# amazon-science/crossmodal-contrastive-learning

Hardware: AMD Instinct MI355X
Metric: contrastive-pairs/sec (fwd+bwd) (higher is better)
Workload: dtype bf16

## Files before the change

### crossmodal-contrastive-learning_amd/csrc/crossclr_api.cpp

```cpp
#include "../../include/crossclr.h"
#include "crossclr_kernels_generic.h"
#include "crossclr_kernels_hvp.h"
#include "crossclr_kernels_topk.h"
#ifndef CROSSCLR_NO_FAST
#include "crossclr_kernels_fast.h"
#include "crossclr_kernels_project.h"
#include "crossclr_kernels_saved32.h"
#endif

#include <math.h>
#include <stdarg.h>
#include <stdio.h>
#include <stdlib.h>
#include <string.h>
#include <type_traits>

#ifndef CROSSCLR_DEFAULT_BWD_KERNEL
#define CROSSCLR_DEFAULT_BWD_KERNEL 1
#endif

using namespace crossclr;

static thread_local char g_err[512] = "";

// ... 265 lines not shown

template <typename TIN, bool NORM>
static int normalize_t(const crossclr_plan* p, const void* v, const void* t, long ldv, long ldt, void* xhat,
                       float* inv_norm, float* diag, void* stream, int* zero_word) {
    Geo g; memset(&g, 0, sizeof(g));
    g.b = p->b; g.bpad = p->bpad; g.D = p->D; g.Dpad = p->Dpad;
    dim3 grid((p->bpad + 3) / 4), block(256);
    if (p->mode == CROSSCLR_MODE_FP32)
        LAUNCH((normalize_kernel<TIN, float, NORM>), grid, block, stream, (const TIN*)v, (const TIN*)t, ldv, ldt, g,
               (float*)xhat, inv_norm, diag, zero_word);
    else if (is_x3(p))
        LAUNCH((normalize_kernel<TIN, x3_t, NORM>), grid, block, stream, (const TIN*)v, (const TIN*)t, ldv, ldt, g,
               (x3_t*)xhat, inv_norm, diag, zero_word);
    else
        LAUNCH((normalize_kernel<TIN, bf16_t, NORM>), grid, block, stream, (const TIN*)v, (const TIN*)t, ldv, ldt, g,
               (bf16_t*)xhat, inv_norm, diag, zero_word);
    return launch_status("normalize_kernel");
}
template <bool NORM>
static int normalize_any(const crossclr_plan* plan, const void* video, const void* text, long ld_video, long ld_text, int in_dtype,
                         void* xhat, float* inv_norm, float* diag_cos, void* stream, int* zero_word = nullptr) {
    if (!plan || !video || !text || !xhat || !inv_norm || !diag_cos) return fail(CROSSCLR_E_ARG, "NULL argument");
    if (ld_video < plan->D || ld_text < plan->D) return fail(CROSSCLR_E_ARG, "row stride smaller than D");
    switch (in_dtype) {
        case CROSSCLR_IN_F32: return normalize_t<float, NORM>(plan, video, text, ld_video, ld_text, xhat, inv_norm, diag_cos, stream, zero_word);
        case CROSSCLR_IN_F64: return normalize_t<double, NORM>(plan, video, text, ld_video, ld_text, xhat, inv_norm, diag_cos, stream, zero_word);
        case CROSSCLR_IN_F16: return normalize_t<in_f16, NORM>(plan, video, text, ld_video, ld_text, xhat, inv_norm, diag_cos, stream, zero_word);
        case CROSSCLR_IN_BF16: return normalize_t<in_bf16, NORM>(plan, video, text, ld_video, ld_text, xhat, inv_norm, diag_cos, stream, zero_word);
    }
    return fail(CROSSCLR_E_ARG, "bad in_dtype %d", in_dtype);
}

#ifndef CROSSCLR_NO_FAST
template <typename TIN, bool NORM>
static int normalize_xf_t(const crossclr_plan* p, const void* v, const void* t, long ldv, long ldt, void* xhat, void* xf,
                          float* inv_norm, float* diag, void* stream, int* zero_word) {
    Geo g; memset(&g, 0, sizeof(g));
    g.b = p->b; g.bpad = p->bpad; g.D = p->D; g.Dpad = p->Dpad;
    if (p->Dpad <= 512)
        LAUNCH((normalize_xf_kernel<TIN, NORM, 2>), dim3(p->bpad / 16), dim3(512), stream, (const TIN*)v, (const TIN*)t, ldv, ldt, g,
               (bf16_t*)xhat, (unsigned char*)xf, inv_norm, diag, zero_word);
    else
        LAUNCH((normalize_xf_kernel<TIN, NORM, 4>), dim3(p->bpad / 16), dim3(512), stream, (const TIN*)v, (const TIN*)t, ldv, ldt, g,
               (bf16_t*)xhat, (unsigned char*)xf, inv_norm, diag, zero_word);
    return launch_status("normalize_xf_kernel");
}
#endif
template <bool NORM>
static int normalize_xf_any(const crossclr_plan* plan, const void* video, const void* text, long ld_video, long ld_text, int in_dtype,
                            void* xhat, void* xf, float* inv_norm, float* diag_cos, void* stream, int* zero_word = nullptr) {
    if (!plan || !video || !text || !xhat || !xf || !inv_norm || !diag_cos) return fail(CROSSCLR_E_ARG, "NULL argument");
    if (ld_video < plan->D || ld_text < plan->D) return fail(CROSSCLR_E_ARG, "row stride smaller than D");
#ifdef CROSSCLR_NO_FAST
    return fail(CROSSCLR_E_ARG, "the fragment-major operand needs the register-resident path");
#else
    if (!plan->xf_bytes) return fail(CROSSCLR_E_ARG, "this plan has no fragment-major operand (xf_bytes == 0): use crossclr_normalize / crossclr_pack");
    if (plan->Dpad > 1024) {
        if (int rc = normalize_any<NORM>(plan, video, text, ld_video, ld_text, in_dtype, xhat, inv_norm, diag_cos, stream, zero_word)) return rc;
        return crossclr_pack_xf_from_packed(plan, xhat, 1, xf, stream);
    }
    switch (in_dtype) {
        case CROSSCLR_IN_F32: return normalize_xf_t<float, NORM>(plan, video, text, ld_video, ld_text, xhat, xf, inv_norm, diag_cos, stream, zero_word);
        case CROSSCLR_IN_F64: return normalize_xf_t<double, NORM>(plan, video, text, ld_video, ld_text, xhat, xf, inv_norm, diag_cos, stream, zero_word);
        case CROSSCLR_IN_F16: return normalize_xf_t<in_f16, NORM>(plan, video, text, ld_video, ld_text, xhat, xf, inv_norm, diag_cos, stream, zero_word);
        case CROSSCLR_IN_BF16: return normalize_xf_t<in_bf16, NORM>(plan, video, text, ld_video, ld_text, xhat, xf, inv_norm, diag_cos, stream, zero_word);
    }
    return fail(CROSSCLR_E_ARG, "bad in_dtype %d", in_dtype);
#endif
}
extern "C" int crossclr_normalize_xf(const crossclr_plan* plan, const void* video, const void* text, long ld_video, long ld_text,
                                     int in_dtype, void* xhat, void* xhat_xf, float* inv_norm, float* diag_cos, void* stream) {
    return normalize_xf_any<true>(plan, video, text, ld_video, ld_text, in_dtype, xhat, xhat_xf, inv_norm, diag_cos, stream);
}
extern "C" int crossclr_pack_xf(const crossclr_plan* plan, const void* video_hat, const void* text_hat, long ld_video, long ld_text,
                                int in_dtype, void* xhat, void* xhat_xf, float* inv_norm, float* diag_cos, void* stream) {
    return normalize_xf_any<false>(plan, video_hat, text_hat, ld_video, ld_text, in_dtype, xhat, xhat_xf, inv_norm, diag_cos, stream);
}
// ... 433 lines not shown
        return fail(CROSSCLR_E_ARG, "slot0 must be L * plan->fwd_slots, L = 0..%d", kLaunchGroups - 1);
    const int n = 2 * plan->bpad;
    LAUNCH(fwd_add_kernel, dim3((n + 255) / 256), dim3(256), stream, vec, n, part + (size_t)slot0 * n,
           reinterpret_cast<int*>(part + ws_flag_off(plan)) + 4 * (slot0 / plan->fwd_slots));
    return launch_status("fwd_add_kernel");
}

extern "C" int crossclr_forward_finish(const crossclr_plan* plan, const float* part, int nslots,
                                       const float* diag_cos, float temperature, float negative_weight,
                                       float* logz, float* rz, float* wrz, double* loss_sum, void* stream) {
    return crossclr_forward_finish_w(plan, part, nslots, diag_cos, temperature, negative_weight, nullptr, logz, rz, wrz,
                                     loss_sum, stream);
}

extern "C" int crossclr_forward_finish_w(const crossclr_plan* plan, const float* part, int nslots,
                                         const float* diag_cos, float temperature, float negative_weight,
                                         const crossclr_sample_weights* sw, float* logz, float* rz, float* wrz,
                                         double* loss_sum, void* stream) {
    if (!plan || !part || !diag_cos || !logz || !rz || !wrz || !loss_sum || plan->fwd_slots <= 0 || nslots <= 0 ||
        nslots % plan->fwd_slots != 0 || nslots / plan->fwd_slots > kLaunchGroups)
        return fail(CROSSCLR_E_ARG, "NULL argument / nslots must be fwd_slots times the number of launch groups (1..%d)", kLaunchGroups);
    Geo g;
    int rc = make_geo(plan, 1, plan->rank, -1, temperature, negative_weight, &g);
    if (rc) return rc;
    const int nb = plan->loss_ws_doubles - 1;
    const int nlaunch = nslots / plan->fwd_slots;
    return crossclr_forward_finish_s(plan, part, nslots, diag_cos, temperature, negative_weight, sw, nullptr, logz, rz, wrz, loss_sum,
                                     stream);
}

static int forward_finish_impl(const crossclr_plan* plan, const float* part, int nslots,
                               const float* diag_cos, float temperature, float negative_weight,
                               const crossclr_sample_weights* sw, const float* shift_rows, float* logz, float* rz,
                               float* wrz, double* loss_sum, void* stream, int* ticket);
extern "C" int crossclr_forward_finish_s(const crossclr_plan* plan, const float* part, int nslots,
                                         const float* diag_cos, float temperature, float negative_weight,
                                         const crossclr_sample_weights* sw, const float* shift_rows, float* logz, float* rz,
                                         float* wrz, double* loss_sum, void* stream) {
    return forward_finish_impl(plan, part, nslots, diag_cos, temperature, negative_weight, sw, shift_rows, logz, rz, wrz, loss_sum, stream, nullptr);
}
static int forward_finish_impl(const crossclr_plan* plan, const float* part, int nslots,
                               const float* diag_cos, float temperature, float negative_weight,
                               const crossclr_sample_weights* sw, const float* shift_rows, float* logz, float* rz,
                               float* wrz, double* loss_sum, void* stream, int* ticket) {
    if (!plan || !part || !diag_cos || !logz || !rz || !wrz || !loss_sum || plan->fwd_slots <= 0 || nslots <= 0 ||
        nslots % plan->fwd_slots != 0 || nslots / plan->fwd_slots > kLaunchGroups)
        return fail(CROSSCLR_E_ARG, "NULL argument / nslots must be fwd_slots times the number of launch groups (1..%d)", kLaunchGroups);
    Geo g;
    int rc = make_geo(plan, 1, plan->rank, -1, temperature, negative_weight, &g, shift_rows != nullptr);
    if (rc) return rc;
    if ((g.row_shift != 0) != (shift_rows != nullptr))
        return fail(CROSSCLR_E_ARG, "shift_rows must be given exactly when crossclr_needs_row_shift(temperature, negative_weight)");
    const int nb = plan->loss_ws_doubles - 1;
    const int nlaunch = nslots / plan->fwd_slots;
    LAUNCH(fwd_finish_kernel, dim3(nb), dim3(256), stream, part, nlaunch, plan->fwd_slots, g, diag_cos, 1.0f / temperature,
           negative_weight, logz, rz, wrz, loss_sum, part + ws_colpart_off(plan),
           reinterpret_cast<const int*>(part + ws_flag_off(plan)), sw ? sw->neg_scale_rows : nullptr,
           sw ? sw->loss_weight : nullptr, shift_rows, ticket, 1.0 / (2.0 * (double)plan->b * (double)plan->world));
    if (!ticket) LAUNCH(fwd_finish_reduce_kernel, dim3(1), dim3(64), stream, loss_sum, nb, 1.0 / (2.0 * (double)plan->b * (double)plan->world));
    return launch_status("fwd_finish_kernel");
}

extern "C" int crossclr_needs_row_shift(float temperature, float negative_weight) {
    return (temperature > 0.f && isfinite(temperature) && isfinite(negative_weight) && needs_row_shift(temperature, negative_weight)) ? 1 : 0;
}

extern "C" int crossclr_forward_rowmax(const crossclr_plan* plan, const void* xhat_rows, const void* xhat_cols, int col_ranks,
                                       int col_rank0, int skip_rank, float temperature, float negative_weight,
                                       const crossclr_sample_weights* sw, float* part, float* shift_rows, int accumulate,
                                       void* stream) {
    if (!plan || !xhat_rows || !xhat_cols || !part || !shift_rows) return fail(CROSSCLR_E_ARG, "NULL argument");
    const float *krows, *kcols;
    if (int rk = unpack_k(sw, &krows, &kcols)) return rk;
    Geo g;
    int rc = make_geo(plan, col_ranks, col_rank0, skip_rank, temperature, negative_weight, &g, true);
    if (rc) return rc;
    const bool skipping = skip_rank >= col_rank0 && skip_rank < col_rank0 + col_ranks;
    const int n = 2 * plan->bpad;
    int nslots = plan->fwd_slots;
    const float* colpart = nullptr;
    if (col_ranks - (skipping ? 1 : 0) <= 0) nslots = 0;
    else if (xhat_rows == xhat_cols && col_ranks == 1 && col_rank0 == plan->rank && skip_rank < 0 && krows == kcols &&
             !env_knobs().disable_symmetric) {
        float* cp = part + ws_colpart_off(plan);
        int* header = reinterpret_cast<int*>(part + ws_flag_off(plan));
        rc = is_x3(plan) ? forward_generic_sym<x3_t>(plan, g, xhat_rows, part, kcols, cp, header, stream, nullptr, nullptr, true)
           : plan->mode == CROSSCLR_MODE_FP32 ? forward_generic_sym<float>(plan, g, xhat_rows, part, kcols, cp, header, stream, nullptr, nullptr, true)
                                              : forward_generic_sym<bf16_t>(plan, g, xhat_rows, part, kcols, cp, header, stream, nullptr, nullptr, true);
        if (rc) return rc;
        colpart = cp;
    } else if ((rc = forward_generic(plan, g, xhat_rows, xhat_cols, part, kcols, nullptr, 1, stream))) return rc;
// ... 1063 lines not shown
    if (int rc = step_bind(plan, layout, persistent, transient, true, &B)) return rc;
    const crossclr_step_layout& L = B.L;
    const float temperature = L.temperature, negative_weight = L.negative_weight;
    const unsigned flags = L.flags;
    const float* k = sw ? sw->neg_scale_rows : nullptr;
    const float* lw = sw ? sw->loss_weight : nullptr;
    const crossclr_sample_weights sw_k = {k, k, nullptr}, sw_klw = {k, k, lw};
    const crossclr_sample_weights* pk = k ? &sw_k : nullptr;
    const crossclr_sample_weights* pklw = (k || lw) ? &sw_klw : nullptr;
    const bool pre = (flags & CROSSCLR_STEP_PRENORMALIZED) != 0;
    int rc;
    int* ticket = reinterpret_cast<int*>(B.at(L.ticket));
    if (L.xf != CROSSCLR_STEP_NONE)
        rc = pre ? normalize_xf_any<false>(plan, video, text, ld_video, ld_text, in_dtype, B.xhat(), B.v(L.xf), B.f(L.inv_norm), B.f(L.diag), stream, ticket)
                 : normalize_xf_any<true>(plan, video, text, ld_video, ld_text, in_dtype, B.xhat(), B.v(L.xf), B.f(L.inv_norm), B.f(L.diag), stream, ticket);
    else
        rc = pre ? normalize_any<false>(plan, video, text, ld_video, ld_text, in_dtype, B.xhat(), B.f(L.inv_norm), B.f(L.diag), stream, ticket)
                 : normalize_any<true>(plan, video, text, ld_video, ld_text, in_dtype, B.xhat(), B.f(L.inv_norm), B.f(L.diag), stream, ticket);
    if (rc) return rc;
    if (L.two_pass) {
        rc = crossclr_forward_rowmax(plan, B.xhat(), B.xhat(), 1, plan->rank, -1, temperature, negative_weight, pk, B.f(L.part), B.f(L.shift), 0, stream);
        if (rc) return rc;
        rc = L.saved ? crossclr_forward_save_s(plan, B.xhat(), temperature, negative_weight, pk, B.f(L.shift), B.f(L.part), 0, B.v(L.stash), stream)
                     : crossclr_forward_s(plan, B.xhat(), B.xhat(), 1, plan->rank, -1, temperature, negative_weight, pk, B.f(L.shift), B.f(L.part), 0, stream);
        if (rc) return rc;
        rc = forward_finish_impl(plan, B.f(L.part), plan->fwd_slots, B.f(L.diag), temperature, negative_weight, pklw, B.f(L.shift),
                                 B.f(L.logz), B.f(L.rz), B.f(L.wrz), loss_ws, stream, ticket);
        if (rc || L.gbuf == CROSSCLR_STEP_NONE) return rc;
        return step_gradient_product(plan, B, k, B.f(L.gbuf), L.saved != 0, stream);
    }
    rc = L.saved ? crossclr_forward_save(plan, B.xhat(), temperature, negative_weight, pk, B.f(L.part), 0, B.v(L.stash), stream)
                 : crossclr_forward_w(plan, B.xhat(), B.xhat(), 1, plan->rank, -1, temperature, negative_weight, pk, B.f(L.part), 0, stream);
    if (rc) return rc;
    rc = forward_finish_impl(plan, B.f(L.part), plan->fwd_slots, B.f(L.diag), temperature, negative_weight, pklw, nullptr, B.f(L.logz), B.f(L.rz),
                             B.f(L.wrz), loss_ws, stream, ticket);
    if (rc || L.gbuf == CROSSCLR_STEP_NONE) return rc;
    return step_gradient_product(plan, B, k, B.f(L.gbuf), L.saved != 0, stream);
}

static int step_gradient_product(const crossclr_plan* plan, const StepBufs& B, const float* k, float* gbuf, bool from_saved, void* stream) {
    const crossclr_step_layout& L = B.L;
    const float temperature = L.temperature, negative_weight = L.negative_weight;
    const crossclr_sample_weights sw_k = {k, k, nullptr};
    const crossclr_sample_weights* pk = k ? &sw_k : nullptr;
    float *rz = B.f(L.rz), *wrz = B.f(L.wrz);
    if (L.two_pass)
        return from_saved ? crossclr_backward_saved_s(plan, B.xhat(), B.v(L.stash), temperature, negative_weight, rz, wrz, pk, gbuf, 0, stream)
                          : crossclr_backward_s(plan, B.xhat(), B.xhat(), 1, plan->rank, -1, temperature, negative_weight, rz, wrz, rz, wrz, pk,
                                                B.f(L.shift), B.f(L.shift), gbuf, 0, stream);
    if (from_saved) {
        switch (L.backward_kernel) {
            case 3: return crossclr_backward_saved_xfp(plan, B.v(L.xf), B.v(L.stash), temperature, negative_weight, rz, wrz, pk, gbuf, 0, stream);
            case 2: return crossclr_backward_saved_xf(plan, B.v(L.xf), B.v(L.stash), temperature, negative_weight, rz, wrz, pk, gbuf, 0, stream);
            default: return crossclr_backward_saved(plan, B.xhat(), B.v(L.stash), temperature, negative_weight, rz, wrz, pk, gbuf, 0, stream);
        }
    }
    return crossclr_backward_w(plan, B.xhat(), B.xhat(), 1, plan->rank, -1, temperature, negative_weight, rz, wrz, rz, wrz, pk, gbuf, 0, stream);
}

extern "C" int crossclr_step_backward(const crossclr_plan* plan, const crossclr_step_layout* layout, const void* video, const void* text,
                                      long ld_video, long ld_text, int in_dtype, const crossclr_sample_weights* sw,
                                      void* persistent, void* transient, void* scratch, const double* grad_out,
                                      void* grad_video, void* grad_text, long ld_gvideo, long ld_gtext, void* stream) {
    if (!video || !text || !grad_out || !grad_video || !grad_text) return fail(CROSSCLR_E_ARG, "NULL argument");
    StepBufs B;
    if (int rc = step_bind(plan, layout, persistent, transient, false, &B)) return rc;
    const crossclr_step_layout& L = B.L;
    if (L.flags & CROSSCLR_STEP_FORWARD_ONLY) return fail(CROSSCLR_E_ARG, "the forward of this step was declared CROSSCLR_STEP_FORWARD_ONLY");
// ... 186 lines not shown
```

### crossmodal-contrastive-learning_amd/csrc/crossclr_kernels_generic.h

```cpp
#pragma once
#include "crossclr_device.h"

namespace crossclr {

struct in_f16 { unsigned short bits; };
struct in_bf16 { unsigned short bits; };
__device__ __forceinline__ double in_load(const float* p, size_t i) { return (double)p[i]; }
__device__ __forceinline__ double in_load(const double* p, size_t i) { return p[i]; }
__device__ __forceinline__ double in_load(const in_bf16* p, size_t i) { return (double)bf16_bits_to_f32(p[i].bits); }
__device__ __forceinline__ double in_load(const in_f16* p, size_t i) {
    return (double)(float)__builtin_bit_cast(_Float16, p[i].bits);
}
__device__ __forceinline__ void in_store(float* p, size_t i, double v) { p[i] = (float)v; }
__device__ __forceinline__ void in_store(double* p, size_t i, double v) { p[i] = v; }
__device__ __forceinline__ void in_store(in_bf16* p, size_t i, double v) { p[i].bits = f32_to_bf16_bits((float)v); }
__device__ __forceinline__ void in_store(in_f16* p, size_t i, double v) {
    p[i].bits = __builtin_bit_cast(unsigned short, (_Float16)(float)v);
}
__device__ __forceinline__ void op_store(float* p, size_t i, float v) { p[i] = v; }
__device__ __forceinline__ void op_store(bf16_t* p, size_t i, float v) { p[i] = f32_to_bf16_bits(v); }
__device__ __forceinline__ void op_store(x3_t* p, size_t i, float v) {
    bf16_t h, l;
    x3_split(v, &h, &l);
    unsigned char* c = reinterpret_cast<unsigned char*>(p) + (i >> 5) * 128 + (i & 31) * 2;
// ... 104 lines not shown
        }
    }
    ssv = wave_sum_f64(ssv); sst = wave_sum_f64(sst); dot = wave_sum_f64(dot);
    double nv = sqrt(ssv), nt = sqrt(sst);
    double iv = 1.0 / (nv > 1e-12 ? nv : 1e-12), it = 1.0 / (nt > 1e-12 ? nt : 1e-12);
    if (!NORM) iv = it = 1.0;
    if (cached) {
#pragma unroll
        for (int k = 0; k < kRowCache; ++k) {
            const int d = 4 * lane + 256 * k;
            if (d < g.Dpad) {
                float a[4] = {0.f, 0.f, 0.f, 0.f}, c[4] = {0.f, 0.f, 0.f, 0.f};
                if (d < g.D) {
#pragma unroll
                    for (int j = 0; j < 4; ++j) { a[j] = (float)(cv[k][j] * iv); c[j] = (float)(ct[k][j] * it); }
                }
                op_store4(xv, d, a); op_store4(xt, d, c);
            }
        }
        for (int d = 4 * lane + 256 * kRowCache; d < g.Dpad; d += 256) { op_store4(xv, d, zero4); op_store4(xt, d, zero4); }
    } else {
        for (int d = lane; d < g.Dpad; d += 64) {
            float a = 0.f, c = 0.f;
            if (d < g.D) { a = (float)(in_load(pv, d) * iv); c = (float)(in_load(pt, d) * it); }
            op_store(xv, d, a); op_store(xt, d, c);
        }
    }
    if (lane == 0) {
        inv_norm[i] = (float)iv; inv_norm[g.bpad + i] = (float)it;
        diag_cos[i] = (float)(dot * iv * it);
    }
}

template <typename TIN, bool NORM, int KC>
__global__ void __launch_bounds__(512) normalize_xf_kernel(const TIN* video, const TIN* text, long ldv, long ldt, Geo g, bf16_t* X,
                                                           unsigned char* XF, float* inv_norm, float* diag_cos, int* zero_word) {
    CROSSCLR_SHARED __attribute__((aligned(16))) bf16_t sh[2][16][256 * KC];
    if (zero_word && blockIdx.x == 0 && threadIdx.x == 0) *zero_word = 0;
    const int wave = threadIdx.x >> 6, lane = threadIdx.x & 63;
    const int i0 = blockIdx.x * 16;
#pragma unroll
    for (int rr = 0; rr < 2; ++rr) {
        const int r = 2 * wave + rr, i = i0 + r;
        bf16_t* xv = X + (size_t)i * g.Dpad;
        bf16_t* xt = X + ((size_t)g.bpad + i) * g.Dpad;
        double cv[KC][4], ct[KC][4];
        double ssv = 0, sst = 0, dot = 0;
        const bool valid = i < g.b;
        const TIN* pv = video + (size_t)(valid ? i : 0) * ldv;
        const TIN* pt = text + (size_t)(valid ? i : 0) * ldt;
#pragma unroll
        for (int k = 0; k < KC; ++k) {
            const int d = 4 * lane + 256 * k;
#pragma unroll
            for (int j = 0; j < 4; ++j) { cv[k][j] = 0.0; ct[k][j] = 0.0; }
            if (valid && d < g.D) {
                row_load4(pv, d, g.D, cv[k]);
                row_load4(pt, d, g.D, ct[k]);
#pragma unroll
                for (int j = 0; j < 4; ++j) { ssv += cv[k][j] * cv[k][j]; sst += ct[k][j] * ct[k][j]; dot += cv[k][j] * ct[k][j]; }
            }
        }
        ssv = wave_sum_f64(ssv); sst = wave_sum_f64(sst); dot = wave_sum_f64(dot);
        double nv = sqrt(ssv), nt = sqrt(sst);
        double iv = 1.0 / (nv > 1e-12 ? nv : 1e-12), it = 1.0 / (nt > 1e-12 ? nt : 1e-12);
        if (!NORM) iv = it = 1.0;
#pragma unroll
        for (int k = 0; k < KC; ++k) {
            const int d = 4 * lane + 256 * k;
            if (d < g.Dpad) {
                float a[4] = {0.f, 0.f, 0.f, 0.f}, c[4] = {0.f, 0.f, 0.f, 0.f};
                if (valid && d < g.D) {
#pragma unroll
                    for (int j = 0; j < 4; ++j) { a[j] = (float)(cv[k][j] * iv); c[j] = (float)(ct[k][j] * it); }
                }
                op_store4(xv, d, a); op_store4(xt, d, c);
                op_store4(&sh[0][r][0], d, a); op_store4(&sh[1][r][0], d, c);
            }
        }
        if (lane == 0) {
            inv_norm[i] = valid ? (float)iv : 0.f; inv_norm[g.bpad + i] = valid ? (float)it : 0.f;
            diag_cos[i] = valid ? (float)(dot * iv * it) : 0.f;
        }
    }
    __syncthreads();
    const int nfr = g.Dpad / 32, ks = (i0 >> 4) & 1;
    for (int c = threadIdx.x; c < 4 * g.Dpad; c += 512) {
        const int m = c / (2 * g.Dpad), rest = c - m * 2 * g.Dpad, h = rest / g.Dpad, d = rest - h * g.Dpad;
        struct { bf16_t e[8]; } v;
#pragma unroll
        for (int e = 0; e < 8; ++e) v.e[e] = sh[m][8 * (e >> 2) + 4 * h + (e & 3)][d];
        const size_t u = ((size_t)m * g.bpad + i0) >> 5;
        *reinterpret_cast<u32x4*>(XF + ((u * nfr + (d >> 5)) * 2 + ks) * 1024 + (32 * h + (d & 31)) * 16) = __builtin_bit_cast(u32x4, v);
    }
}

__global__ void __launch_bounds__(256) xf_from_packed_kernel(const bf16_t* X, unsigned char* XF, int Dpad) {
    CROSSCLR_SHARED __attribute__((aligned(16))) bf16_t sh[32][1024 + 8];
    const size_t u = blockIdx.x;
    const int col0 = blockIdx.y * 1024;
    const int wcols = Dpad - col0 < 1024 ? Dpad - col0 : 1024;
    const bf16_t* src = X + u * 32 * (size_t)Dpad + col0;
    const int chunks = wcols / 8;
    for (int c = threadIdx.x; c < 32 * chunks; c += 256) {
        const int r = c / chunks, k = c - r * chunks;
        *reinterpret_cast<u32x4*>(&sh[r][8 * k]) = *reinterpret_cast<const u32x4*>(src + (size_t)r * Dpad + 8 * k);
    }
    __syncthreads();
    const int nfr = Dpad / 32;
    for (int c = threadIdx.x; c < 4 * wcols; c += 256) {
        const int ks = c / (2 * wcols), rest = c - ks * 2 * wcols, h = rest / wcols, d = rest - h * wcols;
        struct { bf16_t e[8]; } v;
#pragma unroll
        for (int e = 0; e < 8; ++e) v.e[e] = sh[16 * ks + 8 * (e >> 2) + 4 * h + (e & 3)][d];
        const int dg = col0 + d;
        *reinterpret_cast<u32x4*>(XF + ((u * nfr + (dg >> 5)) * 2 + ks) * 1024 + (32 * h + (dg & 31)) * 16) = __builtin_bit_cast(u32x4, v);
    }
}

template <typename T, bool SW, int MODE, bool ST = false, bool SYM = false>
__global__ void __launch_bounds__(256, 2) fwd_sums_kernel(const T* rows, const T* cols, Geo g, int tiles_per_split,
                                                       float* part, const float* kcols, const float* shift, float* stash, int* header,
                                                       float* colpart) {
    static_assert(!ST || MODE == 0 || MODE == 2, "exponentials are saved by the passes that form sums");
    static_assert(!(ST && sizeof(T) == 2) || MODE == 0 || (MODE == 2 && !SYM),
                  "bf16 records: the single-pass forward (symmetric: upper triangle; rectangular: every tile) or the full second pass of the two-pass soft-max");
    static_assert(!SYM || MODE <= 3, "symmetric evaluation: the soft-max passes; MODE 3: one pass for both directions");
// ... 263 lines not shown
        float h = 0.f, c = 0.f;
        if (colpart && p >= bpad) {
            const int nrb = bpad / 128;
            for (int k = 0; k < nrb; ++k) { h += colpart[(size_t)k * n + p]; c += colpart[(size_t)(nrb + k) * n + p]; }
        } else {
            for (int s = 0; s < nslots; ++s) { h += part[(size_t)s * n + p]; c += cnt[(size_t)s * n + p]; }
        }
        const bool valid = (p < bpad ? p : p - bpad) < b;
        hinge[p] = valid ? h : 0.f;
        active[p] = valid ? c : 0.f;
        if (valid) acc += (double)h;
    }
    sh[threadIdx.x] = acc;
    __syncthreads();
    for (int o = 128; o > 0; o >>= 1) {
        if ((int)threadIdx.x < o) sh[threadIdx.x] += sh[threadIdx.x + o];
        __syncthreads();
    }
    if (threadIdx.x == 0) loss_ws[1 + blockIdx.x] = sh[0];
}
__global__ void __launch_bounds__(256) rowmax_combine_kernel(const float* part, int nslots, int n, const float* krows, int accumulate,
                                                             float* shift, const float* colpart) {
    const int p = blockIdx.x * 256 + threadIdx.x;
    if (p >= n) return;
    float m = accumulate ? shift[p] : ((krows && krows[p] == 0.f) ? -3.0e38f : 0.f);
    for (int k = 0; k < nslots; ++k) m = fmaxf(m, part[(size_t)k * n + p]);
    if (colpart) {
        for (int k = 0; k < p / 128; ++k) m = fmaxf(m, colpart[(size_t)k * n + p]);
    }
    shift[p] = m;
}

constexpr int kFinishLpr = 4;
__global__ void __launch_bounds__(256) fwd_finish_kernel(const float* part, int nlaunch, int slots_per_launch, Geo g,
                                                         const float* diag_cos, float inv_tau, float neg_w, float* logz,
                                                         float* rz, float* wrz, double* loss_ws, const float* colpart,
                                                         const int* header, const float* krows, const float* lw,
                                                         const float* row_shift, int* ticket, double scale) {
    CROSSCLR_SHARED double red[4];
    CROSSCLR_SHARED int last_block;
    const int n = 2 * g.bpad;
    double acc = 0.0;
    constexpr int LPR = kFinishLpr;
    const int q = threadIdx.x & (LPR - 1);
    for (int p = (blockIdx.x * 256 + threadIdx.x) / LPR; p < n; p += gridDim.x * (256 / LPR)) {
        const int mod = p / g.bpad, i = p - mod * g.bpad;
        const double shift = (row_shift ? (double)row_shift[p] : (double)g.m2) * (double)kLn2;
        const double self_term = exp(-shift);
        double s = 0.0;
        for (int L = 0; L < nlaunch; ++L) {
            const int kind = header[4 * L], tpr = header[4 * L + 1], NT = header[4 * L + 2], per = header[4 * L + 3];
            const float* base = part + (size_t)L * slots_per_launch * n;
            int count = slots_per_launch;
            if (kind == 0 && tpr != 0) count = tpr > 0 ? tpr : 0;
            if (kind == 4) {
                const int rb = p / (32 * tpr);
#pragma unroll 4
                for (int k = q; k < rb; k += LPR) s += (double)colpart[(size_t)k * n + p];
            } else if (kind != 0) {
                const int rb = p / (32 * tpr);
                count = fwdw_last_block(kind, tpr, NT, per, rb) - fwdw_first_block(kind, tpr, NT, per, rb) + 1;
                if (kind == 1) {
#pragma unroll 4
                    for (int k = q; k < rb; k += LPR) s += (double)colpart[(size_t)k * n + p];
                }
            }
            for (int k = q; k < count; k += LPR) s += (double)base[(size_t)k * n + p];
        }
        s += wave_xor_f64(s, 1);
        s += wave_xor_f64(s, 2);
        if (LPR > 4) { s += wave_xor_f64(s, 4); s += wave_xor_f64(s, 8); }
        s += krows ? self_term * (double)krows[p] : self_term;
        const bool valid = i < g.b;
        const double lz = shift + log(s);
        const double om = lw ? (double)lw[p] : 1.0;
        const float r = valid ? (float)(om / s) : 0.f;
        if (q == 0) {
            logz[p] = valid ? (float)lz : 0.f;
            rz[p] = r;
            wrz[p] = neg_w * r;
            if (valid) {
                acc += om * lz;
                if (mod == 0) acc -= (lw ? om + (double)lw[g.bpad + i] : 2.0) * (double)diag_cos[i] * (double)inv_tau;
            }
        }
    }
    acc = wave_sum_f64(acc);
    if ((threadIdx.x & 63) == 0) red[threadIdx.x >> 6] = acc;
    __syncthreads();
    const double block_sum = (red[0] + red[1]) + (red[2] + red[3]);
    if (ticket == nullptr) {
        if (threadIdx.x == 0) loss_ws[1 + blockIdx.x] = block_sum;
        return;
    }
    if (threadIdx.x == 0) {
        handoff_store_f64(&loss_ws[1 + blockIdx.x], block_sum);
        handoff_stores_complete();
        last_block = atomicAdd(ticket, 1) == (int)gridDim.x - 1;
    }
    __syncthreads();
    if (!last_block || threadIdx.x >= 64) return;
    const int nblocks = (int)gridDim.x;
    double tot = 0.0;
    for (int k = threadIdx.x; k < nblocks; k += 64) tot += handoff_load_f64(&loss_ws[1 + k]);
    tot = wave_sum_f64(tot);
    if (threadIdx.x == 0) { loss_ws[0] = tot; if (nblocks >= 1) loss_ws[1] = tot * scale; *ticket = 0; }
}
__global__ void __launch_bounds__(256) colsum_reduce_kernel(const float* colpart, int nrb, int ncols, float* out) {
    const int c = blockIdx.x * 256 + threadIdx.x;
    if (c >= ncols) return;
    float s = 0.f;
#pragma unroll 8
    for (int rb = 0; rb < nrb; ++rb) s += colpart[(size_t)rb * ncols + c];
    out[c] = s;
}
__global__ void __launch_bounds__(256) fwd_add_kernel(const float* vec, int n, float* slot, int* header) {
// ... 754 lines not shown
```

Before: 153.0 billion.

## Pipeline normalize_xf row loads across persistent blocks and batch loads in forward finish

Result: no change. 153.4 billion, median of 3 (+0.3%).

```diff
diff --git a/crossmodal-contrastive-learning_amd/csrc/crossclr_api.cpp b/crossmodal-contrastive-learning_amd/csrc/crossclr_api.cpp
--- a/crossmodal-contrastive-learning_amd/csrc/crossclr_api.cpp
+++ b/crossmodal-contrastive-learning_amd/csrc/crossclr_api.cpp
@@ -321,17 +321,22 @@
 }
 
 #ifndef CROSSCLR_NO_FAST
+static const int kNormalizeXfBlocks = 256;
 template <typename TIN, bool NORM>
 static int normalize_xf_t(const crossclr_plan* p, const void* v, const void* t, long ldv, long ldt, void* xhat, void* xf,
                           float* inv_norm, float* diag, void* stream, int* zero_word) {
     Geo g; memset(&g, 0, sizeof(g));
     g.b = p->b; g.bpad = p->bpad; g.D = p->D; g.Dpad = p->Dpad;
-    if (p->Dpad <= 512)
-        LAUNCH((normalize_xf_kernel<TIN, NORM, 2>), dim3(p->bpad / 16), dim3(512), stream, (const TIN*)v, (const TIN*)t, ldv, ldt, g,
+    const int nunits = p->bpad / 16;
+    if (p->Dpad <= 512) {
+        const int nblk = normalize_xf_pipelined<TIN, 2>() && nunits > kNormalizeXfBlocks ? kNormalizeXfBlocks : nunits;
+        LAUNCH((normalize_xf_kernel<TIN, NORM, 2>), dim3(nblk), dim3(512), stream, (const TIN*)v, (const TIN*)t, ldv, ldt, g,
                (bf16_t*)xhat, (unsigned char*)xf, inv_norm, diag, zero_word);
-    else
-        LAUNCH((normalize_xf_kernel<TIN, NORM, 4>), dim3(p->bpad / 16), dim3(512), stream, (const TIN*)v, (const TIN*)t, ldv, ldt, g,
+    } else {
+        const int nblk = normalize_xf_pipelined<TIN, 4>() && nunits > kNormalizeXfBlocks ? kNormalizeXfBlocks : nunits;
+        LAUNCH((normalize_xf_kernel<TIN, NORM, 4>), dim3(nblk), dim3(512), stream, (const TIN*)v, (const TIN*)t, ldv, ldt, g,
                (bf16_t*)xhat, (unsigned char*)xf, inv_norm, diag, zero_word);
+    }
     return launch_status("normalize_xf_kernel");
 }
 #endif
@@ -831,17 +836,18 @@
 static int forward_finish_impl(const crossclr_plan* plan, const float* part, int nslots,
                                const float* diag_cos, float temperature, float negative_weight,
                                const crossclr_sample_weights* sw, const float* shift_rows, float* logz, float* rz,
-                               float* wrz, double* loss_sum, void* stream, int* ticket);
+                               float* wrz, double* loss_sum, void* stream, int* ticket, const FinishHint* hint = nullptr);
 extern "C" int crossclr_forward_finish_s(const crossclr_plan* plan, const float* part, int nslots,
                                          const float* diag_cos, float temperature, float negative_weight,
                                          const crossclr_sample_weights* sw, const float* shift_rows, float* logz, float* rz,
                                          float* wrz, double* loss_sum, void* stream) {
     return forward_finish_impl(plan, part, nslots, diag_cos, temperature, negative_weight, sw, shift_rows, logz, rz, wrz, loss_sum, stream, nullptr);
 }
+static_assert(kFinishMaxLaunches >= CROSSCLR_LAUNCH_GROUPS, "fwd_finish_kernel keeps every launch group's header words in LDS");
 static int forward_finish_impl(const crossclr_plan* plan, const float* part, int nslots,
                                const float* diag_cos, float temperature, float negative_weight,
                                const crossclr_sample_weights* sw, const float* shift_rows, float* logz, float* rz,
-                               float* wrz, double* loss_sum, void* stream, int* ticket) {
+                               float* wrz, double* loss_sum, void* stream, int* ticket, const FinishHint* hint) {
     if (!plan || !part || !diag_cos || !logz || !rz || !wrz || !loss_sum || plan->fwd_slots <= 0 || nslots <= 0 ||
         nslots % plan->fwd_slots != 0 || nslots / plan->fwd_slots > kLaunchGroups)
         return fail(CROSSCLR_E_ARG, "NULL argument / nslots must be fwd_slots times the number of launch groups (1..%d)", kLaunchGroups);
@@ -852,10 +858,12 @@
         return fail(CROSSCLR_E_ARG, "shift_rows must be given exactly when crossclr_needs_row_shift(temperature, negative_weight)");
     const int nb = plan->loss_ws_doubles - 1;
     const int nlaunch = nslots / plan->fwd_slots;
+    const FinishHint no_hint = {-1, 0, 0, 0};
     LAUNCH(fwd_finish_kernel, dim3(nb), dim3(256), stream, part, nlaunch, plan->fwd_slots, g, diag_cos, 1.0f / temperature,
            negative_weight, logz, rz, wrz, loss_sum, part + ws_colpart_off(plan),
            reinterpret_cast<const int*>(part + ws_flag_off(plan)), sw ? sw->neg_scale_rows : nullptr,
-           sw ? sw->loss_weight : nullptr, shift_rows, ticket, 1.0 / (2.0 * (double)plan->b * (double)plan->world));
+           sw ? sw->loss_weight : nullptr, shift_rows, ticket, 1.0 / (2.0 * (double)plan->b * (double)plan->world),
+           (hint && nlaunch == 1) ? *hint : no_hint);
     if (!ticket) LAUNCH(fwd_finish_reduce_kernel, dim3(1), dim3(64), stream, loss_sum, nb, 1.0 / (2.0 * (double)plan->b * (double)plan->world));
     return launch_status("fwd_finish_kernel");
 }
@@ -1985,8 +1993,15 @@
     rc = L.saved ? crossclr_forward_save(plan, B.xhat(), temperature, negative_weight, pk, B.f(L.part), 0, B.v(L.stash), stream)
                  : crossclr_forward_w(plan, B.xhat(), B.xhat(), 1, plan->rank, -1, temperature, negative_weight, pk, B.f(L.part), 0, stream);
     if (rc) return rc;
+    FinishHint hint = {-1, 0, 0, 0};
+#ifndef CROSSCLR_NO_FAST
+    if (L.saved && plan->fast_path) {
+        const FwdWork wk = fast_forward_work(plan, 1, -1, true);
+        if (wk.total > 0) hint = FinishHint{wk.kind, wk.tpr, wk.NT, wk.per};
+    }
+#endif
     rc = forward_finish_impl(plan, B.f(L.part), plan->fwd_slots, B.f(L.diag), temperature, negative_weight, pklw, nullptr, B.f(L.logz), B.f(L.rz),
-                             B.f(L.wrz), loss_ws, stream, ticket);
+                             B.f(L.wrz), loss_ws, stream, ticket, hint.kind >= 0 ? &hint : nullptr);
     if (rc || L.gbuf == CROSSCLR_STEP_NONE) return rc;
     return step_gradient_product(plan, B, k, B.f(L.gbuf), L.saved != 0, stream);
 }
diff --git a/crossmodal-contrastive-learning_amd/csrc/crossclr_kernels_generic.h b/crossmodal-contrastive-learning_amd/csrc/crossclr_kernels_generic.h
--- a/crossmodal-contrastive-learning_amd/csrc/crossclr_kernels_generic.h
+++ b/crossmodal-contrastive-learning_amd/csrc/crossclr_kernels_generic.h
@@ -160,57 +160,107 @@
     }
 }
 
-template <typename TIN, bool NORM, int KC>
-__global__ void __launch_bounds__(512) normalize_xf_kernel(const TIN* video, const TIN* text, long ldv, long ldt, Geo g, bf16_t* X,
-                                                           unsigned char* XF, float* inv_norm, float* diag_cos, int* zero_word) {
-    CROSSCLR_SHARED __attribute__((aligned(16))) bf16_t sh[2][16][256 * KC];
-    if (zero_word && blockIdx.x == 0 && threadIdx.x == 0) *zero_word = 0;
-    const int wave = threadIdx.x >> 6, lane = threadIdx.x & 63;
-    const int i0 = blockIdx.x * 16;
-#pragma unroll
-    for (int rr = 0; rr < 2; ++rr) {
-        const int r = 2 * wave + rr, i = i0 + r;
-        bf16_t* xv = X + (size_t)i * g.Dpad;
-        bf16_t* xt = X + ((size_t)g.bpad + i) * g.Dpad;
-        double cv[KC][4], ct[KC][4];
-        double ssv = 0, sst = 0, dot = 0;
-        const bool valid = i < g.b;
-        const TIN* pv = video + (size_t)(valid ? i : 0) * ldv;
-        const TIN* pt = text + (size_t)(valid ? i : 0) * ldt;
-#pragma unroll
-        for (int k = 0; k < KC; ++k) {
-            const int d = 4 * lane + 256 * k;
-#pragma unroll
-            for (int j = 0; j < 4; ++j) { cv[k][j] = 0.0; ct[k][j] = 0.0; }
-            if (valid && d < g.D) {
+template <typename TIN> struct alignas(sizeof(TIN) * 4 > 16 ? 16 : sizeof(TIN) * 4) row_raw4 { TIN e[4]; };
+template <typename TIN>
+__device__ __forceinline__ void row_load4_raw(const TIN* row, int d, int D, row_raw4<TIN>& out) {
+#pragma unroll
+    for (int j = 0; j < 4; ++j)
+        if (d + j < D) out.e[j] = row[d + j];
+}
+template <>
+__device__ __forceinline__ void row_load4_raw<float>(const float* row, int d, int D, row_raw4<float>& out) {
+    if (d + 3 < D && ((reinterpret_cast<uintptr_t>(row + d) & 15) == 0)) {
+        const f32x4 v = *reinterpret_cast<const f32x4*>(row + d);
+#pragma unroll
+        for (int j = 0; j < 4; ++j) out.e[j] = v[j];
+    } else {
+#pragma unroll
+        for (int j = 0; j < 4; ++j)
+            if (d + j < D) out.e[j] = row[d + j];
+    }
+}
+template <typename TIN, int KC, bool VEC>
+__device__ __forceinline__ void xf_pair_load(const TIN* video, const TIN* text, long ldv, long ldt, const Geo& g, int i, int lane,
+                                             row_raw4<TIN> (&rv)[KC], row_raw4<TIN> (&rt)[KC]) {
+    const bool valid = i < g.b;
+    const TIN* pv = video + (size_t)(valid ? i : 0) * ldv;
+    const TIN* pt = text + (size_t)(valid ? i : 0) * ldt;
+#pragma unroll
+    for (int k = 0; k < KC; ++k) {
+        const int d = 4 * lane + 256 * k;
+        const bool in = valid && d < g.D;
+        if (VEC) {
+            rv[k] = *reinterpret_cast<const row_raw4<TIN>*>(pv + (in ? d : 0));
+            rt[k] = *reinterpret_cast<const row_raw4<TIN>*>(pt + (in ? d : 0));
+        } else {
+            rv[k] = row_raw4<TIN>{};
+            rt[k] = row_raw4<TIN>{};
+            if (in) {
+                row_load4_raw(pv, d, g.D, rv[k]);
+                row_load4_raw(pt, d, g.D, rt[k]);
+            }
+        }
+    }
+}
+template <typename TIN, int KC, bool VEC>
+__device__ __forceinline__ void xf_unit_load(const TIN* video, const TIN* text, long ldv, long ldt, const Geo& g, int i0, int wave, int lane,
+                                             row_raw4<TIN> (&rv)[2][KC], row_raw4<TIN> (&rt)[2][KC]) {
+#pragma unroll
+    for (int rr = 0; rr < 2; ++rr) xf_pair_load<TIN, KC, VEC>(video, text, ldv, ldt, g, i0 + 2 * wave + rr, lane, rv[rr], rt[rr]);
+}
+template <typename TIN, int KC> __host__ __device__ constexpr bool normalize_xf_pipelined() { return sizeof(TIN) * KC <= 8; }
+template <typename TIN, bool NORM, int KC, bool DIRECT>
+__device__ __forceinline__ void normalize_xf_pair(const Geo& g, int i, int r, int lane, const row_raw4<TIN> (&rv)[KC], const row_raw4<TIN> (&rt)[KC],
+                                                  const TIN* video, const TIN* text, long ldv, long ldt,
+                                                  bf16_t* X, float* inv_norm, float* diag_cos, bf16_t (&sh)[2][16][256 * KC]) {
+    bf16_t* xv = X + (size_t)i * g.Dpad;
+    bf16_t* xt = X + ((size_t)g.bpad + i) * g.Dpad;
+    double cv[KC][4], ct[KC][4];
+    double ssv = 0, sst = 0, dot = 0;
+    const bool valid = i < g.b;
+    const TIN* pv = video + (size_t)(valid ? i : 0) * ldv;
+    const TIN* pt = text + (size_t)(valid ? i : 0) * ldt;
+#pragma unroll
+    for (int k = 0; k < KC; ++k) {
+        const int d = 4 * lane + 256 * k;
+#pragma unroll
+        for (int j = 0; j < 4; ++j) {
+            cv[k][j] = DIRECT ? 0.0 : in_load(rv[k].e, j);
+            ct[k][j] = DIRECT ? 0.0 : in_load(rt[k].e, j);
+        }
+        if (valid && d < g.D) {
+            if (DIRECT) {
                 row_load4(pv, d, g.D, cv[k]);
                 row_load4(pt, d, g.D, ct[k]);
-#pragma unroll
-                for (int j = 0; j < 4; ++j) { ssv += cv[k][j] * cv[k][j]; sst += ct[k][j] * ct[k][j]; dot += cv[k][j] * ct[k][j]; }
-            }
-        }
-        ssv = wave_sum_f64(ssv); sst = wave_sum_f64(sst); dot = wave_sum_f64(dot);
-        double nv = sqrt(ssv), nt = sqrt(sst);
-        double iv = 1.0 / (nv > 1e-12 ? nv : 1e-12), it = 1.0 / (nt > 1e-12 ? nt : 1e-12);
-        if (!NORM) iv = it = 1.0;
-#pragma unroll
-        for (int k = 0; k < KC; ++k) {
-            const int d = 4 * lane + 256 * k;
-            if (d < g.Dpad) {
-                float a[4] = {0.f, 0.f, 0.f, 0.f}, c[4] = {0.f, 0.f, 0.f, 0.f};
-                if (valid && d < g.D) {
-#pragma unroll
-                    for (int j = 0; j < 4; ++j) { a[j] = (float)(cv[k][j] * iv); c[j] = (float)(ct[k][j] * it); }
-                }
-                op_store4(xv, d, a); op_store4(xt, d, c);
-                op_store4(&sh[0][r][0], d, a); op_store4(&sh[1][r][0], d, c);
-            }
-        }
-        if (lane == 0) {
-            inv_norm[i] = valid ? (float)iv : 0.f; inv_norm[g.bpad + i] = valid ? (float)it : 0.f;
-            diag_cos[i] = valid ? (float)(dot * iv * it) : 0.f;
-        }
-    }
+            }
+#pragma unroll
+            for (int j = 0; j < 4; ++j) { ssv += cv[k][j] * cv[k][j]; sst += ct[k][j] * ct[k][j]; dot += cv[k][j] * ct[k][j]; }
+        }
+    }
+    ssv = wave_sum_f64(ssv); sst = wave_sum_f64(sst); dot = wave_sum_f64(dot);
+    double nrv = sqrt(ssv), nrt = sqrt(sst);
+    double iv = 1.0 / (nrv > 1e-12 ? nrv : 1e-12), it = 1.0 / (nrt > 1e-12 ? nrt : 1e-12);
+    if (!NORM) iv = it = 1.0;
+#pragma unroll
+    for (int k = 0; k < KC; ++k) {
+        const int d = 4 * lane + 256 * k;
+        if (d < g.Dpad) {
+            float a[4] = {0.f, 0.f, 0.f, 0.f}, c[4] = {0.f, 0.f, 0.f, 0.f};
+            if (valid && d < g.D) {
+#pragma unroll
+                for (int j = 0; j < 4; ++j) { a[j] = (float)(cv[k][j] * iv); c[j] = (float)(ct[k][j] * it); }
+            }
+            op_store4(xv, d, a); op_store4(xt, d, c);
+            op_store4(&sh[0][r][0], d, a); op_store4(&sh[1][r][0], d, c);
+        }
+    }
+    if (lane == 0) {
+        inv_norm[i] = valid ? (float)iv : 0.f; inv_norm[g.bpad + i] = valid ? (float)it : 0.f;
+        diag_cos[i] = valid ? (float)(dot * iv * it) : 0.f;
+    }
+}
+template <int KC>
+__device__ __forceinline__ void xf_unit_store(const Geo& g, int i0, unsigned char* XF, bf16_t (&sh)[2][16][256 * KC]) {
     __syncthreads();
     const int nfr = g.Dpad / 32, ks = (i0 >> 4) & 1;
     for (int c = threadIdx.x; c < 4 * g.Dpad; c += 512) {
@@ -221,6 +271,59 @@
         const size_t u = ((size_t)m * g.bpad + i0) >> 5;
         *reinterpret_cast<u32x4*>(XF + ((u * nfr + (d >> 5)) * 2 + ks) * 1024 + (32 * h + (d & 31)) * 16) = __builtin_bit_cast(u32x4, v);
     }
+}
+template <typename TIN, bool NORM, int KC>
+__device__ __forceinline__ void normalize_xf_unit(const Geo& g, int i0, int wave, int lane, const row_raw4<TIN> (&rv)[2][KC],
+                                                  const row_raw4<TIN> (&rt)[2][KC], bf16_t* X, unsigned char* XF, float* inv_norm,
+                                                  float* diag_cos, bf16_t (&sh)[2][16][256 * KC]) {
+#pragma unroll
+    for (int rr = 0; rr < 2; ++rr)
+        normalize_xf_pair<TIN, NORM, KC, false>(g, i0 + 2 * wave + rr, 2 * wave + rr, lane, rv[rr], rt[rr], nullptr, nullptr, 0, 0, X, inv_norm,
+                                                diag_cos, sh);
+    xf_unit_store<KC>(g, i0, XF, sh);
+}
+template <typename TIN, bool NORM, int KC, int NBUF, bool VEC>
+__device__ __forceinline__ void normalize_xf_units(const TIN* video, const TIN* text, long ldv, long ldt, const Geo& g, bf16_t* X, unsigned char* XF,
+                                                   float* inv_norm, float* diag_cos, bf16_t (&sh)[NBUF][2][16][256 * KC]) {
+    const int wave = threadIdx.x >> 6, lane = threadIdx.x & 63;
+    const int nunits = g.bpad / 16, stride = (int)gridDim.x;
+    if constexpr (!normalize_xf_pipelined<TIN, KC>()) {
+        const int unit = blockIdx.x;
+#pragma unroll
+        for (int rr = 0; rr < 2; ++rr) {
+            const row_raw4<TIN> none[KC] = {};
+            normalize_xf_pair<TIN, NORM, KC, true>(g, 16 * unit + 2 * wave + rr, 2 * wave + rr, lane, none, none, video, text, ldv, ldt, X,
+                                                   inv_norm, diag_cos, sh[0]);
+        }
+        xf_unit_store<KC>(g, 16 * unit, XF, sh[0]);
+    } else {
+        row_raw4<TIN> av[2][KC], at[2][KC], bv[2][KC], bt[2][KC];
+        xf_unit_load<TIN, KC, VEC>(video, text, ldv, ldt, g, 16 * (int)blockIdx.x, wave, lane, av, at);
+        xf_unit_load<TIN, KC, VEC>(video, text, ldv, ldt, g, 16 * ((int)blockIdx.x + stride), wave, lane, bv, bt);
+        for (int unit = blockIdx.x; unit < nunits; unit += 2 * stride) {
+            normalize_xf_unit<TIN, NORM, KC>(g, 16 * unit, wave, lane, av, at, X, XF, inv_norm, diag_cos, sh[0]);
+            if (NBUF == 1) __syncthreads();
+            if (unit + stride >= nunits) break;
+            xf_unit_load<TIN, KC, VEC>(video, text, ldv, ldt, g, 16 * (unit + 2 * stride), wave, lane, av, at);
+            normalize_xf_unit<TIN, NORM, KC>(g, 16 * (unit + stride), wave, lane, bv, bt, X, XF, inv_norm, diag_cos, sh[NBUF - 1]);
+            if (NBUF == 1) __syncthreads();
+            xf_unit_load<TIN, KC, VEC>(video, text, ldv, ldt, g, 16 * (unit + 3 * stride), wave, lane, bv, bt);
+        }
+    }
+}
+template <typename TIN, bool NORM, int KC>
+__global__ void __launch_bounds__(512) normalize_xf_kernel(const TIN* video, const TIN* text, long ldv, long ldt, Geo g, bf16_t* X,
+                                                           unsigned char* XF, float* inv_norm, float* diag_cos, int* zero_word) {
+    constexpr int NBUF = (KC <= 2 && normalize_xf_pipelined<TIN, KC>()) ? 2 : 1;
+    CROSSCLR_SHARED __attribute__((aligned(16))) bf16_t sh[NBUF][2][16][256 * KC];
+    if (zero_word && blockIdx.x == 0 && threadIdx.x == 0) *zero_word = 0;
+    constexpr uintptr_t A = alignof(row_raw4<TIN>);
+    const bool vec = g.D % 4 == 0 && (reinterpret_cast<uintptr_t>(video) | reinterpret_cast<uintptr_t>(text) |
+                                      (uintptr_t)ldv * sizeof(TIN) | (uintptr_t)ldt * sizeof(TIN)) % A == 0;
+    if constexpr (normalize_xf_pipelined<TIN, KC>()) {
+        if (vec) { normalize_xf_units<TIN, NORM, KC, NBUF, true>(video, text, ldv, ldt, g, X, XF, inv_norm, diag_cos, sh); return; }
+    }
+    normalize_xf_units<TIN, NORM, KC, NBUF, false>(video, text, ldv, ldt, g, X, XF, inv_norm, diag_cos, sh);
 }
 
 __global__ void __launch_bounds__(256) xf_from_packed_kernel(const bf16_t* X, unsigned char* XF, int Dpad) {
@@ -550,48 +653,73 @@
 }
 
 constexpr int kFinishLpr = 4;
+constexpr int kFinishColCap = 16, kFinishSlotCap = 4;
+constexpr int kFinishMaxLaunches = 8;
+struct FinishHint { int kind, tpr, NT, per; };
 __global__ void __launch_bounds__(256) fwd_finish_kernel(const float* part, int nlaunch, int slots_per_launch, Geo g,
                                                          const float* diag_cos, float inv_tau, float neg_w, float* logz,
                                                          float* rz, float* wrz, double* loss_ws, const float* colpart,
                                                          const int* header, const float* krows, const float* lw,
-                                                         const float* row_shift, int* ticket, double scale) {
+                                                         const float* row_shift, int* ticket, double scale, FinishHint hint) {
     CROSSCLR_SHARED double red[4];
     CROSSCLR_SHARED int last_block;
+    CROSSCLR_SHARED int hdr[4 * kFinishMaxLaunches];
     const int n = 2 * g.bpad;
+    const bool hinted = hint.kind >= 0;
+    if (!hinted) {
+        if ((int)threadIdx.x < 4 * nlaunch) hdr[threadIdx.x] = header[threadIdx.x];
+        __syncthreads();
+    }
     double acc = 0.0;
     constexpr int LPR = kFinishLpr;
     const int q = threadIdx.x & (LPR - 1);
     for (int p = (blockIdx.x * 256 + threadIdx.x) / LPR; p < n; p += gridDim.x * (256 / LPR)) {
         const int mod = p / g.bpad, i = p - mod * g.bpad;
-        const double shift = (row_shift ? (double)row_shift[p] : (double)g.m2) * (double)kLn2;
-        const double self_term = exp(-shift);
+        const bool valid = i < g.b;
+        const float rs_ld = (row_shift ? row_shift : part)[p], kr_ld = (krows ? krows : part)[p], lw_ld = (lw ? lw : part)[p];
+        const float dc = diag_cos[i], lwq = (lw ? lw : part)[g.bpad + i];
+        const float rs = row_shift ? rs_ld : g.m2, kr = krows ? kr_ld : 1.f, lwp = lw ? lw_ld : 1.f;
+        const double shift = (double)rs * (double)kLn2;
+        double self_term = 0.0;
         double s = 0.0;
-        for (int L = 0; L < nlaunch; ++L) {
-            const int kind = header[4 * L], tpr = header[4 * L + 1], NT = header[4 * L + 2], per = header[4 * L + 3];
+        auto launch_terms = [&](int L, bool first) {
+            const int kind = hinted ? hint.kind : hdr[4 * L], tpr = hinted ? hint.tpr : hdr[4 * L + 1];
+            const int NT = hinted ? hint.NT : hdr[4 * L + 2], per = hinted ? hint.per : hdr[4 * L + 3];
             const float* base = part + (size_t)L * slots_per_launch * n;
+            const int rb = kind != 0 ? p / (32 * tpr) : 0;
+            const int ncol = (kind == 1 || kind == 4) ? rb : 0;
+            float cpv[kFinishColCap], slv[kFinishSlotCap];
+#pragma unroll
+            for (int j = 0; j < kFinishColCap; ++j) {
+                const int k = q + LPR * j;
+                cpv[j] = colpart[(size_t)(k < ncol ? k : 0) * n + p];
+            }
             int count = slots_per_launch;
-            if (kind == 0 && tpr != 0) count = tpr > 0 ? tpr : 0;
-            if (kind == 4) {
-                const int rb = p / (32 * tpr);
-#pragma unroll 4
-                for (int k = q; k < rb; k += LPR) s += (double)colpart[(size_t)k * n + p];
-            } else if (kind != 0) {
-                const int rb = p / (32 * tpr);
-                count = fwdw_last_block(kind, tpr, NT, per, rb) - fwdw_first_block(kind, tpr, NT, per, rb) + 1;
-                if (kind == 1) {
-#pragma unroll 4
-                    for (int k = q; k < rb; k += LPR) s += (double)colpart[(size_t)k * n + p];
-                }
-            }
-            for (int k = q; k < count; k += LPR) s += (double)base[(size_t)k * n + p];
-        }
+            if (kind == 0) { if (tpr != 0) count = tpr > 0 ? tpr : 0; }
+            else if (kind != 4) count = fwdw_last_block(kind, tpr, NT, per, rb) - fwdw_first_block(kind, tpr, NT, per, rb) + 1;
+#pragma unroll
+            for (int j = 0; j < kFinishSlotCap; ++j) {
+                const int k = q + LPR * j;
+                slv[j] = base[(size_t)(k < count ? k : 0) * n + p];
+            }
+            if (first) self_term = exp(-shift);
+#pragma unroll
+            for (int j = 0; j < kFinishColCap; ++j)
+                if (q + LPR * j < ncol) s += (double)cpv[j];
+            for (int k = q + LPR * kFinishColCap; k < ncol; k += LPR) s += (double)colpart[(size_t)k * n + p];
+#pragma unroll
+            for (int j = 0; j < kFinishSlotCap; ++j)
+                if (q + LPR * j < count) s += (double)slv[j];
+            for (int k = q + LPR * kFinishSlotCap; k < count; k += LPR) s += (double)base[(size_t)k * n + p];
+        };
+        launch_terms(0, true);
+        for (int L = 1; L < nlaunch; ++L) launch_terms(L, false);
         s += wave_xor_f64(s, 1);
         s += wave_xor_f64(s, 2);
         if (LPR > 4) { s += wave_xor_f64(s, 4); s += wave_xor_f64(s, 8); }
-        s += krows ? self_term * (double)krows[p] : self_term;
-        const bool valid = i < g.b;
+        s += krows ? self_term * (double)kr : self_term;
         const double lz = shift + log(s);
-        const double om = lw ? (double)lw[p] : 1.0;
+        const double om = lw ? (double)lwp : 1.0;
         const float r = valid ? (float)(om / s) : 0.f;
         if (q == 0) {
             logz[p] = valid ? (float)lz : 0.f;
@@ -599,7 +727,7 @@
             wrz[p] = neg_w * r;
             if (valid) {
                 acc += om * lz;
-                if (mod == 0) acc -= (lw ? om + (double)lw[g.bpad + i] : 2.0) * (double)diag_cos[i] * (double)inv_tau;
+                if (mod == 0) acc -= (lw ? om + (double)lwq : 2.0) * (double)dc * (double)inv_tau;
             }
         }
     }
```
